# rampasek/GraphGPS

Measured on NVIDIA H100. Metric: graphs/sec GPSLayer fwd+bwd, higher is better.
Workload: dtype f32

## Files before the change

graphgps_b200/csrc/attention.cu:

```cuda
#include "kernels.cuh"

namespace gps {

namespace {

constexpr int kWarpsPerBlock = 4;

__device__ __forceinline__ int find_graph(const int* __restrict__ gptr, int B, int node) {
  int lo = 0, hi = B;
  while (hi - lo > 1) {
    int mid = (lo + hi) >> 1;
    if (gptr[mid] <= node) lo = mid; else hi = mid;
  }
  return lo;
}

template <int LPR>
__device__ __forceinline__ float group_sum(float v) {
#pragma unroll
  for (int o = LPR / 2; o > 0; o >>= 1) v += __shfl_xor_sync(0xffffffffu, v, o);
  return v;
}

__device__ __forceinline__ int warp_max_i(int v) {
#pragma unroll
  for (int o = 16; o > 0; o >>= 1) v = max(v, __shfl_xor_sync(0xffffffffu, v, o));
  return v;
}

struct DropQuad {
  Philox4 r;
  uint32_t thr;
  float keep_scale;
};
__device__ __forceinline__ void drop_quad_refresh(DropQuad& q, float p, uint64_t seed, uint64_t offset, int head, int i, int jl) {
  q.r = philox4x32(seed, offset + (uint64_t)(GPS_SITE_ATTN_P + head), ((uint64_t)i << 20) | (uint64_t)(jl >> 2));
}
__device__ __forceinline__ float drop_quad_scale(const DropQuad& q, int jl) {
  const int k = jl & 3;
  const uint32_t bits = k == 0 ? q.r.v[0] : k == 1 ? q.r.v[1] : k == 2 ? q.r.v[2] : q.r.v[3];
  return bits >= q.thr ? q.keep_scale : 0.f;
}
__device__ __forceinline__ void drop_quad_init(DropQuad& q, float p) {
  q.thr = (uint32_t)fminf(p * 4294967296.f, 4294967295.f);
  q.keep_scale = 1.f / (1.f - p);
}

template <int CH, int LPR>
__device__ __forceinline__ void load_slice(float4* dst, const float* row, int sub, int nch, bool ok) {
#pragma unroll
  for (int c = 0; c < CH; ++c) {
    int ch = sub + c * LPR;
    dst[c] = (ok && ch < nch) ? ld4(row + ch * 4) : f4zero();
  }
}
template <int CH, int LPR>
__device__ __forceinline__ void store_slice(const float4* src, float* row, int sub, int nch) {
#pragma unroll
  for (int c = 0; c < CH; ++c) {
    int ch = sub + c * LPR;
    if (ch < nch) st4(row + ch * 4, src[c]);
  }
}
template <int CH, int LPR>
__device__ __forceinline__ void store_slice_planes(const float4* src, const Planes& p, int64_t r, int64_t col0, int sub, int nch) {
  if (!p.hi) return;
#pragma unroll
  for (int c = 0; c < CH; ++c) {
    int ch = sub + c * LPR;
    if (ch < nch) planes_store4(p, r, col0 + ch * 4, src[c]);
  }
}
template <int CH>
__device__ __forceinline__ float dot_slice(const float4* a, const float4* b) {
  float s = 0.f;
#pragma unroll
  for (int c = 0; c < CH; ++c) s += a[c].x * b[c].x + a[c].y * b[c].y + a[c].z * b[c].z + a[c].w * b[c].w;
  return s;
}

struct AttnArgs {
  const int* gptr; int B; int N; int H; int hd;
  const float* Q; const float* K; const float* V; int64_t ld;
  float* O; const float* Oc; const float* dO; int64_t ldo;
  float* lse; const float* lsec; float* delta; const float* deltac;
  float* dQ; float* dK; float* dV; int64_t ldg;
  float scale; float p_drop; uint64_t seed, offset;
  const unsigned long long* offset_dev;
  Planes Op, dQp, dKp, dVp;
  int smem_rows;
};
__device__ __forceinline__ uint64_t eff_offset(const AttnArgs& a) {
  return a.offset + ((a.p_drop > 0.f && a.offset_dev) ? *a.offset_dev : 0ull);
}

struct StagedRows {
  const float* x; int64_t ldx;
  const float* y; int64_t ldy;
};
template <int RPB>
__device__ __forceinline__ StagedRows stage_rows(const AttnArgs& a, const float* X, int64_t ldX, const float* Y, int64_t ldY,
                                                 int h, float* sm) {
  const int64_t hoff = (int64_t)h * a.hd;
  StagedRows r{X + hoff, ldX, Y + hoff, ldY};
  const int r0 = blockIdx.x * RPB;
  if (a.smem_rows <= 0 || r0 >= a.N) return r;
  const int last = min(r0 + RPB, a.N) - 1;
  const int kmin = a.gptr[find_graph(a.gptr, a.B, r0)];
  const int R = a.gptr[find_graph(a.gptr, a.B, last) + 1] - kmin;
  if (R > a.smem_rows) return r;
  const int pitch = a.hd + 4, nch = a.hd >> 2;
  float* sx = sm;
  float* sy = sm + (int64_t)a.smem_rows * pitch;
  for (int idx = threadIdx.x; idx < R * nch; idx += blockDim.x) {
    const int row = idx / nch, c = idx - row * nch;
    st4(sx + row * pitch + c * 4, ld4(X + (int64_t)(kmin + row) * ldX + hoff + c * 4));
    st4(sy + row * pitch + c * 4, ld4(Y + (int64_t)(kmin + row) * ldY + hoff + c * 4));
  }
  __syncthreads();
  r.x = sx - (int64_t)kmin * pitch; r.ldx = pitch;
  r.y = sy - (int64_t)kmin * pitch; r.ldy = pitch;
  return r;
}

template <int CH, int LPR>
__global__ void __launch_bounds__(kWarpsPerBlock * 32) k_attn_fwd(AttnArgs a) {
  extern __shared__ float attn_sm[];
  constexpr int RPW = 32 / LPR;
  const int warp = threadIdx.x >> 5, lane = threadIdx.x & 31;
  const int sub = lane % LPR, rloc = lane / LPR;
  const int h = blockIdx.y;
  const int i = (blockIdx.x * kWarpsPerBlock + warp) * RPW + rloc;
  const bool row_ok = i < a.N;
  const int nch = a.hd / 4;
  const uint64_t offs = eff_offset(a);
  int gs = 0, n = 0;
  if (row_ok) {
    int g = find_graph(a.gptr, a.B, i);
    gs = a.gptr[g];
    n = a.gptr[g + 1] - gs;
  }
  const int nloop = warp_max_i(n);
  const int64_t hoff = (int64_t)h * a.hd;
  float4 q[CH], o[CH];
  load_slice<CH, LPR>(q, a.Q + (int64_t)(row_ok ? i : 0) * a.ld + hoff, sub, nch, row_ok);
#pragma unroll
  for (int c = 0; c < CH; ++c) {
    q[c] = f4scale(q[c], a.scale);
    o[c] = f4zero();
  }
  float m = -INFINITY, l = 0.f;
  const bool use_drop = a.p_drop > 0.f;
  DropQuad dq;
  drop_quad_init(dq, a.p_drop);
  const StagedRows kv = stage_rows<RPW * kWarpsPerBlock>(a, a.K, a.ld, a.V, a.ld, h, attn_sm);
  float4 kc[CH], vc[CH];
  load_slice<CH, LPR>(kc, kv.x + (int64_t)gs * kv.ldx, sub, nch, n > 0);
  load_slice<CH, LPR>(vc, kv.y + (int64_t)gs * kv.ldy, sub, nch, n > 0);
  for (int jl = 0; jl < nloop; ++jl) {
    if (use_drop && (jl & 3) == 0) drop_quad_refresh(dq, a.p_drop, a.seed, offs, h, i, jl);
    const bool valid = jl < n;
    const bool nvalid = jl + 1 < n;
    const int jn = gs + (nvalid ? jl + 1 : 0);
    float4 kn[CH], vn[CH];
    load_slice<CH, LPR>(kn, kv.x + (int64_t)jn * kv.ldx, sub, nch, nvalid);
    load_slice<CH, LPR>(vn, kv.y + (int64_t)jn * kv.ldy, sub, nch, nvalid);
    float s = group_sum<LPR>(dot_slice<CH>(q, kc));
    s = valid ? s : -INFINITY;
    const float m_new = fmaxf(m, s);
    const float corr = (m_new == -INFINITY) ? 1.f : __expf(m - m_new);
    const float p = valid ? __expf(s - m_new) : 0.f;
    l = l * corr + p;
    const float pd = use_drop ? p * drop_quad_scale(dq, jl) : p;
#pragma unroll
    for (int c = 0; c < CH; ++c) {
      o[c].x = o[c].x * corr + pd * vc[c].x;
      o[c].y = o[c].y * corr + pd * vc[c].y;
      o[c].z = o[c].z * corr + pd * vc[c].z;
      o[c].w = o[c].w * corr + pd * vc[c].w;
      kc[c] = kn[c];
      vc[c] = vn[c];
    }
    m = m_new;
  }
  if (row_ok) {
    const float inv = 1.f / l;
#pragma unroll
    for (int c = 0; c < CH; ++c) o[c] = f4scale(o[c], inv);
    store_slice<CH, LPR>(o, a.O + (int64_t)i * a.ldo + hoff, sub, nch);
    store_slice_planes<CH, LPR>(o, a.Op, i, hoff, sub, nch);
    if (sub == 0) a.lse[(int64_t)i * a.H + h] = m + __logf(l);
  }
}

__global__ void k_attn_delta(AttnArgs a) {
  const int64_t t = ((int64_t)blockIdx.x * blockDim.x + threadIdx.x) >> 3;
  const int sub = threadIdx.x & 7;
  const bool ok = t < (int64_t)a.N * a.H;
  const int64_t i = ok ? t / a.H : 0;
  const int h = ok ? (int)(t - i * a.H) : 0;
  const float4* go = reinterpret_cast<const float4*>(a.dO + i * a.ldo + (int64_t)h * a.hd);
  const float4* oo = reinterpret_cast<const float4*>(a.Oc + i * a.ldo + (int64_t)h * a.hd);
  float acc = 0.f;
  if (ok)
    for (int c = sub; c < a.hd / 4; c += 8) {
      const float4 x = __ldg(go + c), y = __ldg(oo + c);
      acc += x.x * y.x + x.y * y.y + x.z * y.z + x.w * y.w;
    }
  acc += __shfl_xor_sync(0xffffffffu, acc, 4);
  acc += __shfl_xor_sync(0xffffffffu, acc, 2);
  acc += __shfl_xor_sync(0xffffffffu, acc, 1);
  if (ok && sub == 0) a.delta[t] = acc;
}

template <int CH, int LPR>
__device__ __forceinline__ void attn_bwd_q_body(const AttnArgs& a, float* attn_sm) {
  constexpr int RPW = 32 / LPR;
  const int warp = threadIdx.x >> 5, lane = threadIdx.x & 31;
  const int sub = lane % LPR, rloc = lane / LPR;
  const int h = blockIdx.y;
  const int i = (blockIdx.x * kWarpsPerBlock + warp) * RPW + rloc;
  const bool row_ok = i < a.N;
  const int nch = a.hd / 4;
  const uint64_t offs = eff_offset(a);
  int gs = 0, n = 0;
  if (row_ok) {
    int g = find_graph(a.gptr, a.B, i);
    gs = a.gptr[g];
    n = a.gptr[g + 1] - gs;
  }
  const int nloop = warp_max_i(n);
  const int64_t hoff = (int64_t)h * a.hd;
  const int ir = row_ok ? i : 0;
  float4 q[CH], go[CH], gq[CH];
  load_slice<CH, LPR>(q, a.Q + (int64_t)ir * a.ld + hoff, sub, nch, row_ok);
  load_slice<CH, LPR>(go, a.dO + (int64_t)ir * a.ldo + hoff, sub, nch, row_ok);
  {
    const float dl = row_ok ? a.deltac[(int64_t)i * a.H + h] : 0.f;
#pragma unroll
    for (int c = 0; c < CH; ++c) gq[c] = f4zero();
    const float lse = row_ok ? a.lsec[(int64_t)i * a.H + h] : 0.f;
#pragma unroll
    for (int c = 0; c < CH; ++c) q[c] = f4scale(q[c], a.scale);
    const bool use_drop = a.p_drop > 0.f;
    DropQuad dq;
    drop_quad_init(dq, a.p_drop);
    const StagedRows kv = stage_rows<RPW * kWarpsPerBlock>(a, a.K, a.ld, a.V, a.ld, h, attn_sm);
    float4 kk[CH], vv[CH];
    load_slice<CH, LPR>(kk, kv.x + (int64_t)gs * kv.ldx, sub, nch, n > 0);
    load_slice<CH, LPR>(vv, kv.y + (int64_t)gs * kv.ldy, sub, nch, n > 0);
    for (int jl = 0; jl < nloop; ++jl) {
      if (use_drop && (jl & 3) == 0) drop_quad_refresh(dq, a.p_drop, a.seed, offs, h, i, jl);
      const bool valid = jl < n;
      const bool nvalid = jl + 1 < n;
      const int jn = gs + (nvalid ? jl + 1 : 0);
      float4 kn[CH], vn[CH];
      load_slice<CH, LPR>(kn, kv.x + (int64_t)jn * kv.ldx, sub, nch, nvalid);
      load_slice<CH, LPR>(vn, kv.y + (int64_t)jn * kv.ldy, sub, nch, nvalid);
      float s = dot_slice<CH>(q, kk), dp = dot_slice<CH>(go, vv);
#pragma unroll
      for (int ofs = LPR / 2; ofs > 0; ofs >>= 1) {
        s += __shfl_xor_sync(0xffffffffu, s, ofs);
        dp += __shfl_xor_sync(0xffffffffu, dp, ofs);
      }
      const float p = valid ? __expf(s - lse) : 0.f;
      const float ds = p * (dp * (use_drop ? drop_quad_scale(dq, jl) : 1.f) - dl);
#pragma unroll
      for (int c = 0; c < CH; ++c) {
        gq[c].x += ds * kk[c].x;
        gq[c].y += ds * kk[c].y;
        gq[c].z += ds * kk[c].z;
        gq[c].w += ds * kk[c].w;
        kk[c] = kn[c];
        vv[c] = vn[c];
      }
    }
  }
  if (row_ok) {
#pragma unroll
    for (int c = 0; c < CH; ++c) gq[c] = f4scale(gq[c], a.scale);
    store_slice<CH, LPR>(gq, a.dQ + (int64_t)i * a.ldg + hoff, sub, nch);
    store_slice_planes<CH, LPR>(gq, a.dQp, i, hoff, sub, nch);
  }
}

template <int CH, int LPR>
__device__ __forceinline__ void attn_bwd_kv_body(const AttnArgs& a, float* attn_sm) {
  constexpr int RPW = 32 / LPR;
  const int warp = threadIdx.x >> 5, lane = threadIdx.x & 31;
  const int sub = lane % LPR, rloc = lane / LPR;
  const int h = blockIdx.y;
  const int j = (blockIdx.x * kWarpsPerBlock + warp) * RPW + rloc;
  const bool row_ok = j < a.N;
  const int nch = a.hd / 4;
  const uint64_t offs = eff_offset(a);
  int gs = 0, n = 0;
  if (row_ok) {
    int g = find_graph(a.gptr, a.B, j);
    gs = a.gptr[g];
    n = a.gptr[g + 1] - gs;
  }
  const int nloop = warp_max_i(n);
  const int jl = j - gs;
  const int64_t hoff = (int64_t)h * a.hd;
  const int jr = row_ok ? j : 0;
  float4 kk[CH], vv[CH], gk[CH], gv[CH];
  load_slice<CH, LPR>(kk, a.K + (int64_t)jr * a.ld + hoff, sub, nch, row_ok);
  load_slice<CH, LPR>(vv, a.V + (int64_t)jr * a.ld + hoff, sub, nch, row_ok);
#pragma unroll
  for (int c = 0; c < CH; ++c) {
    gk[c] = f4zero();
    gv[c] = f4zero();
  }
  const StagedRows qd = stage_rows<RPW * kWarpsPerBlock>(a, a.Q, a.ld, a.dO, a.ldo, h, attn_sm);
  float4 q[CH], go[CH];
  load_slice<CH, LPR>(q, qd.x + (int64_t)gs * qd.ldx, sub, nch, n > 0);
  load_slice<CH, LPR>(go, qd.y + (int64_t)gs * qd.ldy, sub, nch, n > 0);
  for (int il = 0; il < nloop; ++il) {
    const bool valid = il < n;
    const int i = gs + (valid ? il : 0);
    const bool nvalid = il + 1 < n;
    const int in_ = gs + (nvalid ? il + 1 : 0);
    float4 qn[CH], gon[CH];
    load_slice<CH, LPR>(qn, qd.x + (int64_t)in_ * qd.ldx, sub, nch, nvalid);
    load_slice<CH, LPR>(gon, qd.y + (int64_t)in_ * qd.ldy, sub, nch, nvalid);
    float s = dot_slice<CH>(q, kk), dp = dot_slice<CH>(go, vv);
#pragma unroll
    for (int ofs = LPR / 2; ofs > 0; ofs >>= 1) {
      s += __shfl_xor_sync(0xffffffffu, s, ofs);
      dp += __shfl_xor_sync(0xffffffffu, dp, ofs);
    }
    const float lse = valid ? a.lsec[(int64_t)i * a.H + h] : 0.f;
    const float dl = valid ? a.deltac[(int64_t)i * a.H + h] : 0.f;
    const float p = valid ? __expf(s * a.scale - lse) : 0.f;
    float dsc = 1.f;
    if (a.p_drop > 0.f) {
      DropQuad dq;
      drop_quad_init(dq, a.p_drop);
      drop_quad_refresh(dq, a.p_drop, a.seed, offs, h, i, jl);
      dsc = drop_quad_scale(dq, jl);
    }
    const float pd = p * dsc;
    const float ds = p * (dp * dsc - dl) * a.scale;
#pragma unroll
    for (int c = 0; c < CH; ++c) {
      gk[c].x += ds * q[c].x; gk[c].y += ds * q[c].y; gk[c].z += ds * q[c].z; gk[c].w += ds * q[c].w;
      gv[c].x += pd * go[c].x; gv[c].y += pd * go[c].y; gv[c].z += pd * go[c].z; gv[c].w += pd * go[c].w;
      q[c] = qn[c];
      go[c] = gon[c];
    }
  }
  if (row_ok) {
    store_slice<CH, LPR>(gk, a.dK + (int64_t)j * a.ldg + hoff, sub, nch);
    store_slice<CH, LPR>(gv, a.dV + (int64_t)j * a.ldg + hoff, sub, nch);
    store_slice_planes<CH, LPR>(gk, a.dKp, j, hoff, sub, nch);
    store_slice_planes<CH, LPR>(gv, a.dVp, j, hoff, sub, nch);
  }
}

template <int CH, int LPR>
__global__ void __launch_bounds__(kWarpsPerBlock * 32) k_attn_bwd(AttnArgs a) {
  extern __shared__ float attn_sm[];
  if (blockIdx.z == 0) attn_bwd_kv_body<CH, LPR>(a, attn_sm);
  else attn_bwd_q_body<CH, LPR>(a, attn_sm);
}

enum { KFWD = 0, KBWD = 1 };

constexpr int kStageBytes = 72 * 1024;

template <int CH, int LPR>
static void launch_one(int which, const AttnArgs& a0, cudaStream_t stream) {
  constexpr int RPW = 32 / LPR;
  AttnArgs a = a0;
  static const bool stage_on = [] {
    const char* e = getenv("GPS_B200_ATTN_STAGE");
    return e && e[0] == '1';
  }();
  const int pitch = a.hd + 4;
  a.smem_rows = (stage_on && a.B > 0 && a.N < 64LL * a.B) ? kStageBytes / (2 * pitch * 4) : 0;
  const size_t smem = a.smem_rows > 0 ? (size_t)2 * a.smem_rows * pitch * 4 : 0;
  static bool attr_done[2] = {false, false};
  if (smem > 0 && !attr_done[which]) {
    if (which == KFWD) cudaFuncSetAttribute(k_attn_fwd<CH, LPR>, cudaFuncAttributeMaxDynamicSharedMemorySize, kStageBytes);
    else cudaFuncSetAttribute(k_attn_bwd<CH, LPR>, cudaFuncAttributeMaxDynamicSharedMemorySize, kStageBytes);
    attr_done[which] = true;
  }
  dim3 grid((unsigned)ceil_div(a.N, (int64_t)RPW * kWarpsPerBlock), (unsigned)a.H, which == KFWD ? 1 : 2);
  dim3 block(kWarpsPerBlock * 32);
  if (which == KFWD) k_attn_fwd<CH, LPR><<<grid, block, smem, stream>>>(a);
  else k_attn_bwd<CH, LPR><<<grid, block, smem, stream>>>(a);
}

static int dispatch(int which, const AttnArgs& a, cudaStream_t stream) {
  GPS_REQUIRE(a.hd > 0 && a.hd % 4 == 0, GPS_ERR_UNSUPPORTED, "attention: head dim %d must be a multiple of 4", a.hd);
  GPS_REQUIRE(a.ld % 4 == 0 && a.ldo % 4 == 0 && (which == KFWD || a.ldg % 4 == 0), GPS_ERR_UNSUPPORTED,
              "attention: leading dimensions must be multiples of 4");
  const int nch = a.hd / 4;
  GPS_REQUIRE(nch <= 48, GPS_ERR_UNSUPPORTED, "attention: head dim %d > 192 not supported", a.hd);
  if (a.N == 0) return GPS_OK;
  int lpr = 1;
  while ((nch + lpr - 1) / lpr > 6) lpr *= 2;
  const int ch = (nch + lpr - 1) / lpr;
#define GPS_ATTN_CASE(CHV, LPRV)                                  \
  if (ch == CHV && lpr == LPRV) {                                 \
    launch_one<CHV, LPRV>(which, a, stream);                      \
    GPS_LAUNCH_CHECK();                                           \
    return GPS_OK;                                                \
  }
  GPS_ATTN_CASE(1, 1) GPS_ATTN_CASE(2, 1) GPS_ATTN_CASE(3, 1) GPS_ATTN_CASE(4, 1) GPS_ATTN_CASE(5, 1)
  GPS_ATTN_CASE(6, 1) GPS_ATTN_CASE(4, 2) GPS_ATTN_CASE(5, 2) GPS_ATTN_CASE(6, 2) GPS_ATTN_CASE(4, 4)
  GPS_ATTN_CASE(5, 4) GPS_ATTN_CASE(6, 4) GPS_ATTN_CASE(4, 8) GPS_ATTN_CASE(5, 8) GPS_ATTN_CASE(6, 8)
#undef GPS_ATTN_CASE
  set_error("attention: no kernel for head dim %d", a.hd);
  return GPS_ERR_UNSUPPORTED;
}

}

int attention_fwd(const GpsGraph& g, int64_t heads, int64_t hd, const float* Q, const float* K, const float* V,
                  int64_t ld, float* O, int64_t ldo, float* lse, float p_drop, uint64_t seed, uint64_t offset,
                  cudaStream_t stream, const unsigned long long* offset_dev, Planes Op) {
  AttnArgs a{};
  a.offset_dev = offset_dev;
  a.Op = Op;
  a.gptr = g.graph_ptr; a.B = (int)g.B; a.N = (int)g.N; a.H = (int)heads; a.hd = (int)hd;
  a.Q = Q; a.K = K; a.V = V; a.ld = ld; a.O = O; a.ldo = ldo; a.lse = lse;
  a.scale = 1.f / sqrtf((float)hd); a.p_drop = p_drop; a.seed = seed; a.offset = offset;
  return dispatch(KFWD, a, stream);
}

int attention_bwd(const GpsGraph& g, int64_t heads, int64_t hd, const float* Q, const float* K, const float* V,
                  int64_t ld, const float* O, const float* dO, int64_t ldo, const float* lse, float* delta,
                  float* dQ, float* dK, float* dV, int64_t ldg, float p_drop, uint64_t seed, uint64_t offset,
                  cudaStream_t stream, const unsigned long long* offset_dev, Planes dQp, Planes dKp, Planes dVp) {
  AttnArgs a{};
  a.offset_dev = offset_dev;
  a.dQp = dQp; a.dKp = dKp; a.dVp = dVp;
  a.gptr = g.graph_ptr; a.B = (int)g.B; a.N = (int)g.N; a.H = (int)heads; a.hd = (int)hd;
  a.Q = Q; a.K = K; a.V = V; a.ld = ld; a.Oc = O; a.dO = dO; a.ldo = ldo; a.lsec = lse;
  a.delta = delta; a.deltac = delta; a.dQ = dQ; a.dK = dK; a.dV = dV; a.ldg = ldg;
  a.scale = 1.f / sqrtf((float)hd); a.p_drop = p_drop; a.seed = seed; a.offset = offset;
  if (a.N == 0) return GPS_OK;
  const int64_t nt = (int64_t)a.N * a.H * 8;
  k_attn_delta<<<(unsigned)ceil_div(nt, (int64_t)256), 256, 0, stream>>>(a);
  GPS_LAUNCH_CHECK();
  return dispatch(KBWD, a, stream);
}

}
```

graphgps_b200/csrc/layer.cu:

```cuda
#include <stdarg.h>
#include <string.h>

#include <algorithm>
#include <atomic>

#include "gemm.cuh"
#include "kernels.cuh"

namespace gps {

int perf_supported(int64_t dim_head, int64_t features);
int64_t perf_mp();
int perf_prep(const float* P, int64_t m, float* Pn, const GpsGraph& g, int64_t H, int* nmax, float* gmax, int* argk,
              cudaStream_t st);
int perf_features_fwd(float* fq, float* fk, const float* Q, const float* K, const GpsGraph& g, int64_t H, int64_t m,
                      float* gmax, int* argq, int* argk, cudaStream_t st);
int perf_linattn_fwd(const GpsGraph& g, int64_t H, int64_t m, const int* nmax, const float* qf, const float* kf,
                     const float* V, const float* gmax, float* O, cudaStream_t st);
int perf_linattn_bwd(const GpsGraph& g, int64_t H, int64_t m, const int* nmax, const float* qf, const float* kf,
                     const float* V, const float* gmax, const float* gO, float* g_qf, float* g_kf, float* gV,
                     float* ggmax, cudaStream_t st);
int perf_features_bwd(float* g_fq, float* g_fk, const float* fq, const float* fk, const float* Q, const float* K,
                      float* gQ, float* gK, const GpsGraph& g, int64_t H, int64_t m, const int* argq, const int* argk,
                      float* ggmax, cudaStream_t st);
// ... 778 lines not shown
    const Planes wp[3] = {P.pq_p, P.pk_p, P.pv_p};
    float* dst[3] = {P.pQ, P.pK, P.pV};
    for (int i = 0; i < 3; ++i)
      GPS_TRY(gemm(linear_fwd(P, N, inner, d, {a->x, d, P.x_p}, {lin[i]->weight, d, wp[i]}, dst[i], inner), sg));
    GPS_TRY(perf_prep(a->perf_proj, P.m, P.pPn, a->graph, P.H, P.pnmax, P.pgmax, P.pargk, sg));
    float* ddst[2] = {P.pfq, P.pfk};
    for (int i = 0; i < 2; ++i)
      GPS_TRY(gemm(linear_fwd(P, NH, P.mp, dh, {dst[i], dh}, {P.pPn, dh}, ddst[i], P.mp), sg));
    GPS_TRY(perf_features_fwd(P.pfq, P.pfk, P.pQ, P.pK, a->graph, P.H, P.m, P.pgmax, P.pargq, P.pargk, sg));
    if (P.perf_pairwise)
      GPS_TRY(perf_quad_fwd(a->graph, P.H, P.m, P.pnmax, P.pfq, P.pfk, P.pV, P.pgmax, P.O, P.pden, sg));
    else
      GPS_TRY(perf_linattn_fwd(a->graph, P.H, P.m, P.pnmax, P.pfq, P.pfk, P.pV, P.pgmax, P.O, sg));
    GemmParams g = linear_fwd(P, N, d, inner, {P.O, inner}, {a->attn_out.weight, inner}, P.hA, d, a->attn_out.bias);
    g.R1 = a->x; g.ldr1 = (int)d; g.stats = stats(BN_A);
    set_dropout(g, P.drop(GPS_SITE_ATTN_OUT));
    g.p_drop2 = P.pa; g.site2 = GPS_SITE_PERF_OUT;
    if (P.nonorm) GPS_TRY(close_with_s(g, sg));
    GPS_TRY(gemm(g, sg));
  }

  if (two_branches) GPS_TRY(sd->order(sd->s3, st));

  if (!P.nonorm) {
    const bool loc = P.gated || P.gine || P.gcn;
    const float* first = loc ? P.xloc : P.hA;
    BnView bf = loc ? bn_view(P, BN_L, a->norm1_local, N) : bn_view(P, BN_A, a->norm1_attn, N);
    const float* second = (loc && (P.attn || P.perf)) ? P.hA : nullptr;
    BnView bs = bn_view(P, BN_A, a->norm1_attn, N);
    GPS_TRY(bn_combine(first, bf, second, bs, P.s, N, d, st, P.s_p));
  }

  {
    GemmParams g = linear_fwd(P, N, 2 * d, d, {P.s, d, P.s_p}, {a->ff1.weight, d, P.ff1_p}, P.hid, 2 * d, a->ff1.bias);
    g.act = act; g.C_pre = P.hid_pre; g.ldpre = (int)(2 * d); g.Cp = P.hid_p;
    set_dropout(g, P.drop(GPS_SITE_FF1));
    GPS_TRY(gemm(g, st));
    GemmParams g2 = linear_fwd(P, N, d, 2 * d, {P.hid, 2 * d, P.hid_p}, {a->ff2.weight, 2 * d, P.ff2_p}, P.t, d,
                               a->ff2.bias);
    g2.R1 = P.s; g2.ldr1 = (int)d; g2.stats = stats(BN_2);
    set_dropout(g2, P.drop(GPS_SITE_FF2));
    if (P.nonorm) {
      g2.C = a->x_out;
      g2.Cp = out_planes(a->x_planes_out);
    }
    GPS_TRY(gemm(g2, st));
    if (!P.nonorm)
      GPS_TRY(bn_combine(P.t, bn_view(P, BN_2, a->norm2, N), nullptr, BnView(), a->x_out, N, d, st,
                         out_planes(a->x_planes_out)));
  }
  return GPS_OK;
}

static int layer_backward(const GpsLayerArgs* a, cudaStream_t st) {
  Plan P;
  GPS_TRY(make_plan(a, &P, true));
  GPS_REQUIRE(a->saved && a->workspace, GPS_ERR_ARG, "saved/workspace buffers are required");
  GPS_REQUIRE(a->workspace_bytes >= P.bwd_bytes, GPS_ERR_ARG, "workspace too small (%lld < %lld)",
              (long long)a->workspace_bytes, (long long)P.bwd_bytes);
  GPS_TRY(check_params(a, P));
  GPS_REQUIRE(a->grad_x_out && a->grad_x, GPS_ERR_ARG, "grad_x_out / grad_x are required");
  const int64_t N = P.N, E = P.E, d = P.d;
  const int act = a->act;
  DropCfg nodrop;
  auto sums = [&](int which) { return P.bsums + (int64_t)which * 2 * d; };
  GPS_CUDA(cudaMemsetAsync(P.bsums, 0, (size_t)P.nbn * 2 * d * sizeof(double), st));
  Side* sd;
  GPS_TRY(side_stream(&sd));
  cudaStream_t s2 = sd->s;
  auto wfork = [&](cudaStream_t from) -> int { return sd->order(from, s2); };
  const bool two_branches = (P.gated || P.gine || P.gcn) && (P.attn || P.perf);
  cudaStream_t sa = two_branches ? sd->s3 : st;
  cudaStream_t se = sd->s4;
  const int opt = opt_flags();
  auto record_ev = [&](void* ev, cudaStream_t s) -> int {
    if (!ev) return GPS_OK;
    cudaStreamCaptureStatus cs = cudaStreamCaptureStatusNone;
    GPS_CUDA(cudaStreamIsCapturing(s, &cs));
    GPS_CUDA(cudaEventRecordWithFlags((cudaEvent_t)ev, s, cs == cudaStreamCaptureStatusActive ? cudaEventRecordExternal
                                                                                               : cudaEventRecordDefault));
    return GPS_OK;
  };
  auto early_done = [&]() -> int { return record_ev(a->ev_grads_early, s2); };
  auto mid_done = [&]() -> int { return record_ev(a->ev_grads_mid, s2); };
  const bool gx_splitk = P.Wy >= 1024 && N > 0;
  if (P.Wy) {
    GPS_TRY(wfork(st));
    GPS_CUDA(cudaMemsetAsync(P.gWcat, 0, (size_t)(P.Wy * d + P.Wy) * sizeof(float), s2));
  }
  if (gx_splitk) GPS_CUDA(cudaMemsetAsync(a->grad_x, 0, (size_t)(N * d) * sizeof(float), st));

  if (P.gated) {
    GPS_TRY(sd->order(st, se));
    BnView ve = bn_view(P, BN_E, a->bn_edge_e);
    if (a->grad_edge_out && E > 0) {
      GPS_TRY(bn_bwd_reduce(a->grad_edge_out, d, P.ehat, d, E, d, ve, act, P.drop(GPS_SITE_GCN_E), sums(BN_E), se));
      GPS_TRY(bn_bwd_apply(a->grad_edge_out, d, P.ehat, d, E, d, ve, act, P.drop(GPS_SITE_GCN_E), sums(BN_E), P.g_e, d,
                           a->bn_edge_e.grad_weight, a->bn_edge_e.grad_bias, se, P.grads_accumulate));
    } else {
      if (E > 0) GPS_CUDA(cudaMemsetAsync(P.g_e, 0, (size_t)(E * d) * sizeof(float), se));
      if (a->bn_edge_e.grad_weight && !P.grads_prezeroed)
        GPS_CUDA(cudaMemsetAsync(a->bn_edge_e.grad_weight, 0, d * sizeof(float), se));
      if (a->bn_edge_e.grad_bias && !P.grads_prezeroed)
        GPS_CUDA(cudaMemsetAsync(a->bn_edge_e.grad_bias, 0, d * sizeof(float), se));
    }
  }

  const float* g_t = P.nonorm ? a->grad_x_out : P.g_t;
  if (!P.nonorm) {
    BnView v2 = bn_view(P, BN_2, a->norm2);
    GPS_TRY(bn_bwd_reduce(a->grad_x_out, d, P.t, d, N, d, v2, -1, nodrop, sums(BN_2), st));
    GPS_TRY(bn_bwd_apply(a->grad_x_out, d, P.t, d, N, d, v2, -1, nodrop, sums(BN_2), P.g_t, d, a->norm2.grad_weight,
                         a->norm2.grad_bias, st, P.grads_accumulate, P.gt_p));
  } else if (!(P.dropout.p > 0.f) && P.gt_p.hi && N > 0) {
    ToPlanesItem it{g_t, d, (int)N, (int)d, P.gt_p};
    GPS_TRY(to_planes(&it, 1, st));
  }
  const float* g_xloc = P.nonorm ? P.g_s : P.g_xloc;
  const Planes g_xloc_p = P.nonorm ? P.gs_p : P.gl1_p;
  const float* g_hA = P.nonorm ? P.g_s : P.g_hA;
  const Planes g_hA_p = P.nonorm ? P.gs_p : P.ghA_p;

  bool fused_la = false;
  {
    Operand g_ff2;
    GPS_TRY(dropmul(P, {g_t, d, P.gt_p}, P.g_tmp, P.gtmp_p, GPS_SITE_FF2, st, &g_ff2));
    GemmParams g = linear_dgrad(P, N, 2 * d, d, g_ff2, {a->ff2.weight, 2 * d, P.ff2_p}, P.g_hid, 2 * d);
    set_act_mask(g, act, P.hid, P.hid_pre, 2 * d);
    set_dropout(g, P.drop(GPS_SITE_FF1));
    g.Cp = P.ghid_p;
    GPS_TRY(gemm(g, st));
    const Operand g_hid{P.g_hid, 2 * d, P.ghid_p};
    GPS_TRY(wfork(st));
    GPS_TRY(linear_wgrad(P, g_ff2, {P.hid, 2 * d, P.hid_p}, N, d, 2 * d, a->ff2.grad_weight, a->ff2.grad_bias, s2));
    GPS_TRY(linear_wgrad(P, g_hid, {P.s, d, P.s_p}, N, 2 * d, d, a->ff1.grad_weight, a->ff1.grad_bias, s2));
    GemmParams g2 = linear_dgrad(P, N, d, 2 * d, g_hid, {a->ff1.weight, d, P.ff1_p}, P.g_s, d);
    g2.R1 = g_t; g2.ldr1 = (int)d;
    g2.Cp = P.gs_p;
    fused_la = (opt & 64) && !P.nonorm && P.use_planes && g2.Ap.hi && g2.Bp.hi && N > 0 && P.train;
    if (fused_la) {
      if (P.gated || P.gine || P.gcn) {
        BnView v = bn_view(P, BN_L, a->norm1_local);
        g2.bnred[0].z = P.xloc; g2.bnred[0].ldz = (int)d; g2.bnred[0].mean = v.mean; g2.bnred[0].invstd = v.invstd;
        g2.bnred[0].sums = sums(BN_L);
      }
      if (P.attn || P.perf) {
        BnView v = bn_view(P, BN_A, a->norm1_attn);
        g2.bnred[1].z = P.hA; g2.bnred[1].ldz = (int)d; g2.bnred[1].mean = v.mean; g2.bnred[1].invstd = v.invstd;
        g2.bnred[1].sums = sums(BN_A);
      }
    }
    GPS_TRY(gemm(g2, st));
  }

  const bool loc = P.gated || P.gine || P.gcn;
  bool chain_x = false;
  if (loc && !P.nonorm) {
    BnView v = bn_view(P, BN_L, a->norm1_local);
    if (!fused_la) GPS_TRY(bn_bwd_reduce(P.g_s, d, P.xloc, d, N, d, v, -1, nodrop, sums(BN_L), st));
    chain_x = P.gated && N > 0 && (opt & 32) && P.train;
    if (chain_x)
      GPS_TRY(bn_bwd_apply_chain(P.g_s, d, P.xloc, d, N, d, v, sums(BN_L), P.g_xloc, d, a->norm1_local.grad_weight,
                                 a->norm1_local.grad_bias, P.grads_accumulate, P.gl1_p, P.xt, d,
                                 bn_view(P, BN_X, a->bn_node_x), act, P.drop(GPS_SITE_GCN_X), sums(BN_X), st));
    else
      GPS_TRY(bn_bwd_apply(P.g_s, d, P.xloc, d, N, d, v, -1, nodrop, sums(BN_L), P.g_xloc, d,
                           a->norm1_local.grad_weight, a->norm1_local.grad_bias, st, P.grads_accumulate, P.gl1_p));
  }
  if (!P.attn && !P.perf) {
    GPS_TRY(wfork(st));
    GPS_TRY(early_done());
  }
  if (two_branches) GPS_TRY(sd->order(st, sa));
  if (P.attn) {
    if (!P.nonorm) {
      BnView v = bn_view(P, BN_A, a->norm1_attn);
      if (!fused_la) GPS_TRY(bn_bwd_reduce(P.g_s, d, P.hA, d, N, d, v, -1, nodrop, sums(BN_A), sa));
      GPS_TRY(bn_bwd_apply(P.g_s, d, P.hA, d, N, d, v, -1, nodrop, sums(BN_A), P.g_hA, d, a->norm1_attn.grad_weight,
                           a->norm1_attn.grad_bias, sa, P.grads_accumulate, P.ghA_p));
    }
    Operand g_ao;
    GPS_TRY(dropmul(P, {g_hA, d, g_hA_p}, P.g_tmp2, P.gtmp2_p, GPS_SITE_ATTN_OUT, sa, &g_ao));
    GPS_TRY(gemm(linear_dgrad(P, N, d, d, g_ao, {a->attn_out.weight, d, P.out_p}, P.g_O, d), sa));
    GPS_TRY(wfork(sa));
    GPS_TRY(linear_wgrad(P, g_ao, {P.O, d, P.O_p}, N, d, d, a->attn_out.grad_weight, a->attn_out.grad_bias, s2));
    GPS_TRY(early_done());
    const float* Q = P.Y1 + P.qkv_off;
    float* gQ = P.gY1 + P.qkv_off;
    GPS_TRY(attention_bwd(a->graph, P.H, P.hd, Q, Q + d, Q + 2 * d, P.Wy, P.O, P.g_O, d, P.lse, P.delta, gQ, gQ + d,
                          gQ + 2 * d, P.Wy, P.pa, a->seed, a->offset, sa, (const unsigned long long*)a->offset_dev,
                          P.gY1_p.cols(P.qkv_off), P.gY1_p.cols(P.qkv_off + d), P.gY1_p.cols(P.qkv_off + 2 * d)));
  }

  if (P.perf) {
    const int64_t inner = P.inner, NH = N * P.H, dh = a->perf_dim_head;
    if (!P.nonorm) {
      BnView v = bn_view(P, BN_A, a->norm1_attn);
      if (!fused_la) GPS_TRY(bn_bwd_reduce(P.g_s, d, P.hA, d, N, d, v, -1, nodrop, sums(BN_A), sa));
      GPS_TRY(bn_bwd_apply(P.g_s, d, P.hA, d, N, d, v, -1, nodrop, sums(BN_A), P.g_hA, d, a->norm1_attn.grad_weight,
                           a->norm1_attn.grad_bias, sa, P.grads_accumulate));
    }
    Operand g_ao;
    GPS_TRY(dropmul(P, {g_hA, d}, P.g_tmp2, Planes(), GPS_SITE_ATTN_OUT, sa, &g_ao, P.pa, GPS_SITE_PERF_OUT));
    GPS_TRY(gemm(linear_dgrad(P, N, inner, d, g_ao, {a->attn_out.weight, inner}, P.g_O, inner), sa));
    GPS_TRY(wfork(sa));
    GPS_TRY(linear_wgrad(P, g_ao, {P.O, inner}, N, d, inner, a->attn_out.grad_weight, a->attn_out.grad_bias, s2));
    GPS_TRY(early_done());
    if (P.perf_pairwise)
      GPS_TRY(perf_quad_bwd(a->graph, P.H, P.m, P.pnmax, P.pfq, P.pfk, P.pV, P.pgmax, P.O, P.pden, P.g_O, P.g_pden,
                            P.g_pfq, P.g_pfk, P.g_pV, P.g_pgmax, sa));
    else
      GPS_TRY(perf_linattn_bwd(a->graph, P.H, P.m, P.pnmax, P.pfq, P.pfk, P.pV, P.pgmax, P.g_O, P.g_pfq, P.g_pfk, P.g_pV,
                               P.g_pgmax, sa));
    GPS_TRY(perf_features_bwd(P.g_pfq, P.g_pfk, P.pfq, P.pfk, P.pQ, P.pK, P.g_pQ, P.g_pK, a->graph, P.H, P.m, P.pargq,
                              P.pargk, P.g_pgmax, sa));
    float* gdd[2] = {P.g_pfq, P.g_pfk};
    float* gqk[2] = {P.g_pQ, P.g_pK};
    for (int i = 0; i < 2; ++i) {
      GemmParams h = linear_dgrad(P, NH, dh, P.mp, {gdd[i], P.mp}, {P.pPn, dh}, gqk[i], dh);
      h.R1 = gqk[i]; h.ldr1 = (int)dh;
      GPS_TRY(gemm(h, sa));
    }
    const GpsLinear* lin[3] = {&a->perf_q, &a->perf_k, &a->perf_v};
    const float* gsrc[3] = {P.g_pQ, P.g_pK, P.g_pV};
    GPS_TRY(wfork(sa));
    for (int i = 0; i < 3; ++i) {
      GPS_TRY(linear_wgrad(P, {gsrc[i], inner}, {a->x, d}, N, inner, d, lin[i]->grad_weight, nullptr, s2));
      GemmParams h = linear_dgrad(P, N, d, inner, {gsrc[i], inner}, {lin[i]->weight, d}, P.g_xp, d);
      h.R1 = i == 0 ? g_hA : P.g_xp; h.ldr1 = (int)d;
      GPS_TRY(gemm(h, sa));
    }
  }

  const float* g_x_local = nullptr;
  if (P.gated) {
    BnView vx = bn_view(P, BN_X, a->bn_node_x);
    if (!chain_x)
      GPS_TRY(bn_bwd_reduce(g_xloc, d, P.xt, d, N, d, vx, act, P.drop(GPS_SITE_GCN_X), sums(BN_X), st));
    GPS_TRY(bn_bwd_apply(g_xloc, d, P.xt, d, N, d, vx, act, P.drop(GPS_SITE_GCN_X), sums(BN_X), P.gY1, P.Wy,
                         a->bn_node_x.grad_weight, a->bn_node_x.grad_bias, st, P.grads_accumulate, P.gY1_p));
    GPS_TRY(sd->order(se, st));
    GPS_TRY(gatedgcn_bwd_dst(a->graph, d, P.gY1, P.Wy, P.ehat, P.Y1 + d, P.Wy, P.g_e, P.g_num, P.gY1 + 2 * d, st, P.ge_p,
                             P.gY1_p.cols(2 * d), P.pe_rho, P.g_den));
    if (P.eslap) {
      GPS_TRY(sd->order(st, se));
      GPS_TRY(eslap_bwd(a->graph, a->pe, a->pe_dim, d, act, P.g_num, P.g_den, P.Y1 + d, P.Wy, P.ehat, P.pe_r, P.pe_rho,
                        a->pe_mlp0.weight, a->pe_mlp0.bias, a->pe_mlp1.weight, P.pe_gz, P.pe_gr, P.pe_part, a->grad_pe,
                        a->pe_mlp0.grad_weight, a->pe_mlp0.grad_bias, a->pe_mlp1.grad_weight, a->pe_mlp1.grad_bias,
                        P.grads_accumulate, se));
    }
    GPS_TRY(gatedgcn_bwd_src(a->graph, d, P.g_e, P.ehat, P.g_num, P.gY1 + 3 * d, P.gY1 + d, P.Wy, st, P.gY1_p.cols(3 * d),
                             P.gY1_p.cols(d), P.pe_rho));
    const Operand g_e{P.g_e, d, P.ge_p};
    GPS_TRY(wfork(st));
    GPS_TRY(linear_wgrad(P, g_e, {a->edge_attr, d, P.e_p}, E, d, d, a->gcn_C.grad_weight, a->gcn_C.grad_bias, s2));
    if (P.eslap) GPS_TRY(sd->order(se, s2));
    GPS_TRY(mid_done());
    if (a->grad_edge_attr && E > 0) {
      GemmParams g = linear_dgrad(P, E, d, d, g_e, {a->gcn_C.weight, d, P.C_p}, a->grad_edge_attr, d);
      g.R1 = a->grad_edge_out; g.ldr1 = (int)d;
      GPS_TRY(gemm(g, st));
    }
    g_x_local = g_xloc;
  } else if (P.gine) {
    Operand g_l1;
    GPS_TRY(dropmul(P, {g_xloc, d, g_xloc_p}, P.g_tmp3, P.gtmp3_p, GPS_SITE_LOCAL, st, &g_l1));
    GemmParams g = linear_dgrad(P, N, d, d, g_l1, {a->gine_lin1.weight, d, P.g1_p}, P.g_h1, d);
    set_act_mask(g, act, P.h1, P.h1_pre, d);
    g.Cp = P.gh1_p;
    GPS_TRY(gemm(g, st));
    const Operand g_h1{P.g_h1, d, P.gh1_p};
    GPS_TRY(wfork(st));
    GPS_TRY(linear_wgrad(P, g_l1, {P.h1, d, P.h1_p}, N, d, d, a->gine_lin1.grad_weight, a->gine_lin1.grad_bias, s2));
    GPS_TRY(linear_wgrad(P, g_h1, {P.agg, d, P.agg_p}, N, d, d, a->gine_lin0.grad_weight, a->gine_lin0.grad_bias, s2));
    GPS_TRY(mid_done());
    GPS_TRY(gemm(linear_dgrad(P, N, d, d, g_h1, {a->gine_lin0.weight, d, P.g0_p}, P.g_agg, d), st));
    GPS_REQUIRE(a->grad_edge_attr || E == 0, GPS_ERR_ARG, "grad_edge_attr is required for GINE");
    GPS_TRY(gine_bwd_dst(a->graph, d, a->x, a->edge_attr, P.g_agg, a->grad_edge_attr, st));
    GPS_TRY(gine_bwd_src(a->graph, d, a->grad_edge_attr, P.g_agg, a->gine_eps, g_xloc, P.g_xl, st));
    g_x_local = P.g_xl;
  } else if (P.gcn) {
    Operand g_h;
    GPS_TRY(dropmul(P, {g_xloc, d}, P.g_tmp3, Planes(), GPS_SITE_LOCAL, st, &g_h));
    if (a->gcn_conv.grad_bias) {
      if (!P.grads_prezeroed) GPS_CUDA(cudaMemsetAsync(a->gcn_conv.grad_bias, 0, (size_t)d * sizeof(float), st));
      GPS_TRY(colsum(g_h.f, d, N, d, a->gcn_conv.grad_bias, st));
    }
    GPS_TRY(gcn_bwd(a->graph, d, g_h.f, P.dinv, P.gY1, P.Wy, st, P.gY1_p));
    GPS_TRY(wfork(st));
    GPS_TRY(mid_done());
    g_x_local = g_xloc;
  }

  if (two_branches) GPS_TRY(sd->order(sa, st));

  if (P.Wy) {
    const Operand gY1{P.gY1, P.Wy, P.gY1_p};
    GPS_TRY(wfork(st));
    GPS_TRY(wgrad_add(P, gY1, {a->x, d, P.x_p}, N, P.Wy, d, P.gWcat, P.gbcat, s2));
    PackDesc pdsc = pack_desc(P);
    k_unpack<<<(unsigned)P.Wy, 128, 0, s2>>>(pdsc, P.gWcat, P.gbcat, P.grads_accumulate ? 1 : 0);
    GPS_LAUNCH_CHECK();
    GemmParams g = linear_dgrad(P, N, d, P.Wy, gY1, {P.Wcat, d, P.Wcat_p}, a->grad_x, d);
    g.R1 = g_x_local; g.ldr1 = (int)d;
    g.R2 = P.attn ? g_hA : (P.perf ? P.g_xp : nullptr); g.ldr2 = (int)d;
    if (gx_splitk) g.splitk = 4;
    GPS_TRY(gemm(g, st));
  } else if (g_x_local) {
    GPS_TRY(add3(g_x_local, d, P.perf ? P.g_xp : nullptr, d, nullptr, 0, a->grad_x, d, N, d, st));
  } else {
    GPS_TRY(add3(P.g_xp, d, nullptr, 0, nullptr, 0, a->grad_x, d, N, d, st));
  }
  GPS_TRY(sd->join(st));
  GPS_TRY(record_ev(a->ev_grads_done, st));
  return GPS_OK;
}

}

using namespace gps;

extern "C" const char* gps_last_error(void) { return g_err; }
extern "C" int gps_abi_version(void) { return GPS_ABI_VERSION; }
extern "C" const char* gps_build_arch(void) { return "sm_90a"; }
extern "C" unsigned long long gps_launch_count(void) { return g_launches.load(); }
extern "C" unsigned long long gps_fallback_count(void) { return g_fallbacks.load(); }
// ... 233 lines not shown
```

Measured before the change: 338,900.

## Add fused shared-memory attention backward kernel for small graphs

```diff
diff --git a/graphgps_b200/csrc/attention.cu b/graphgps_b200/csrc/attention.cu
--- a/graphgps_b200/csrc/attention.cu
+++ b/graphgps_b200/csrc/attention.cu
@@ -6,13 +6,15 @@
 
 constexpr int kWarpsPerBlock = 4;
 
-__device__ __forceinline__ int find_graph(const int* __restrict__ gptr, int B, int node) {
-  int lo = 0, hi = B;
+__device__ __forceinline__ int find_graph_in(const int* __restrict__ gptr, int lo, int hi, int node) {
   while (hi - lo > 1) {
     int mid = (lo + hi) >> 1;
     if (gptr[mid] <= node) lo = mid; else hi = mid;
   }
   return lo;
+}
+__device__ __forceinline__ int find_graph(const int* __restrict__ gptr, int B, int node) {
+  return find_graph_in(gptr, 0, B, node);
 }
 
 template <int LPR>
@@ -214,13 +216,8 @@
 }
 
 template <int CH, int LPR>
-__device__ __forceinline__ void attn_bwd_q_body(const AttnArgs& a, float* attn_sm) {
-  constexpr int RPW = 32 / LPR;
-  const int warp = threadIdx.x >> 5, lane = threadIdx.x & 31;
-  const int sub = lane % LPR, rloc = lane / LPR;
-  const int h = blockIdx.y;
-  const int i = (blockIdx.x * kWarpsPerBlock + warp) * RPW + rloc;
-  const bool row_ok = i < a.N;
+__device__ __forceinline__ void attn_bwd_q_body(const AttnArgs& a, int h, int i, bool row_ok) {
+  const int sub = (threadIdx.x & 31) % LPR;
   const int nch = a.hd / 4;
   const uint64_t offs = eff_offset(a);
   int gs = 0, n = 0;
@@ -245,18 +242,19 @@
     const bool use_drop = a.p_drop > 0.f;
     DropQuad dq;
     drop_quad_init(dq, a.p_drop);
-    const StagedRows kv = stage_rows<RPW * kWarpsPerBlock>(a, a.K, a.ld, a.V, a.ld, h, attn_sm);
+    const float* Kh = a.K + hoff;
+    const float* Vh = a.V + hoff;
     float4 kk[CH], vv[CH];
-    load_slice<CH, LPR>(kk, kv.x + (int64_t)gs * kv.ldx, sub, nch, n > 0);
-    load_slice<CH, LPR>(vv, kv.y + (int64_t)gs * kv.ldy, sub, nch, n > 0);
+    load_slice<CH, LPR>(kk, Kh + (int64_t)gs * a.ld, sub, nch, n > 0);
+    load_slice<CH, LPR>(vv, Vh + (int64_t)gs * a.ld, sub, nch, n > 0);
     for (int jl = 0; jl < nloop; ++jl) {
       if (use_drop && (jl & 3) == 0) drop_quad_refresh(dq, a.p_drop, a.seed, offs, h, i, jl);
       const bool valid = jl < n;
       const bool nvalid = jl + 1 < n;
       const int jn = gs + (nvalid ? jl + 1 : 0);
       float4 kn[CH], vn[CH];
-      load_slice<CH, LPR>(kn, kv.x + (int64_t)jn * kv.ldx, sub, nch, nvalid);
-      load_slice<CH, LPR>(vn, kv.y + (int64_t)jn * kv.ldy, sub, nch, nvalid);
+      load_slice<CH, LPR>(kn, Kh + (int64_t)jn * a.ld, sub, nch, nvalid);
+      load_slice<CH, LPR>(vn, Vh + (int64_t)jn * a.ld, sub, nch, nvalid);
       float s = dot_slice<CH>(q, kk), dp = dot_slice<CH>(go, vv);
 #pragma unroll
       for (int ofs = LPR / 2; ofs > 0; ofs >>= 1) {
@@ -285,13 +283,8 @@
 }
 
 template <int CH, int LPR>
-__device__ __forceinline__ void attn_bwd_kv_body(const AttnArgs& a, float* attn_sm) {
-  constexpr int RPW = 32 / LPR;
-  const int warp = threadIdx.x >> 5, lane = threadIdx.x & 31;
-  const int sub = lane % LPR, rloc = lane / LPR;
-  const int h = blockIdx.y;
-  const int j = (blockIdx.x * kWarpsPerBlock + warp) * RPW + rloc;
-  const bool row_ok = j < a.N;
+__device__ __forceinline__ void attn_bwd_kv_body(const AttnArgs& a, int h, int j, bool row_ok) {
+  const int sub = (threadIdx.x & 31) % LPR;
   const int nch = a.hd / 4;
   const uint64_t offs = eff_offset(a);
   int gs = 0, n = 0;
@@ -312,18 +305,19 @@
     gk[c] = f4zero();
     gv[c] = f4zero();
   }
-  const StagedRows qd = stage_rows<RPW * kWarpsPerBlock>(a, a.Q, a.ld, a.dO, a.ldo, h, attn_sm);
+  const float* Qh = a.Q + hoff;
+  const float* dOh = a.dO + hoff;
   float4 q[CH], go[CH];
-  load_slice<CH, LPR>(q, qd.x + (int64_t)gs * qd.ldx, sub, nch, n > 0);
-  load_slice<CH, LPR>(go, qd.y + (int64_t)gs * qd.ldy, sub, nch, n > 0);
+  load_slice<CH, LPR>(q, Qh + (int64_t)gs * a.ld, sub, nch, n > 0);
+  load_slice<CH, LPR>(go, dOh + (int64_t)gs * a.ldo, sub, nch, n > 0);
   for (int il = 0; il < nloop; ++il) {
     const bool valid = il < n;
     const int i = gs + (valid ? il : 0);
     const bool nvalid = il + 1 < n;
     const int in_ = gs + (nvalid ? il + 1 : 0);
     float4 qn[CH], gon[CH];
-    load_slice<CH, LPR>(qn, qd.x + (int64_t)in_ * qd.ldx, sub, nch, nvalid);
-    load_slice<CH, LPR>(gon, qd.y + (int64_t)in_ * qd.ldy, sub, nch, nvalid);
+    load_slice<CH, LPR>(qn, Qh + (int64_t)in_ * a.ld, sub, nch, nvalid);
+    load_slice<CH, LPR>(gon, dOh + (int64_t)in_ * a.ldo, sub, nch, nvalid);
     float s = dot_slice<CH>(q, kk), dp = dot_slice<CH>(go, vv);
 #pragma unroll
     for (int ofs = LPR / 2; ofs > 0; ofs >>= 1) {
@@ -360,12 +354,176 @@
 
 template <int CH, int LPR>
 __global__ void __launch_bounds__(kWarpsPerBlock * 32) k_attn_bwd(AttnArgs a) {
+  constexpr int RPW = 32 / LPR;
+  const int i = (blockIdx.x * kWarpsPerBlock + (threadIdx.x >> 5)) * RPW + (threadIdx.x & 31) / LPR;
+  if (blockIdx.z == 0) attn_bwd_kv_body<CH, LPR>(a, blockIdx.y, i, i < a.N);
+  else attn_bwd_q_body<CH, LPR>(a, blockIdx.y, i, i < a.N);
+}
+
+__host__ __device__ constexpr int bwd_small_pitch(int hd) { return ((hd >> 2) & 1) ? hd : hd + 4; }
+__host__ __device__ constexpr int64_t bwd_small_smem_bytes(int hd, int rows) {
+  return 4 * ((int64_t)rows * (4 * bwd_small_pitch(hd) + hd / 4 + 2) + 2LL * rows * (rows + 1));
+}
+constexpr int kBwdSmallSmemBytes = 44 * 1024;
+
+__device__ __forceinline__ int warp_first_above(const int* __restrict__ gptr, int lo, int hi, int x) {
+  const int lane = threadIdx.x & 31;
+  while (hi > lo) {
+    const int step = (hi - lo + 30) / 31;
+    const unsigned above = __ballot_sync(0xffffffffu, gptr[min(lo + lane * step, hi)] > x);
+    const int f = __ffs(above) - 1;
+    if (f == 0) return lo;
+    hi = min(lo + f * step, hi);
+    lo += (f - 1) * step + 1;
+  }
+  return lo;
+}
+
+__device__ __forceinline__ float dot4(float4 a, float4 b) { return a.x * b.x + a.y * b.y + a.z * b.z + a.w * b.w; }
+__device__ __forceinline__ float4 f4axpy(float w, float4 x, float4 y) {
+  return make_float4(fmaf(w, x.x, y.x), fmaf(w, x.y, y.y), fmaf(w, x.z, y.z), fmaf(w, x.w, y.w));
+}
+
+template <int LPR>
+__global__ void __launch_bounds__(kWarpsPerBlock * 32) k_attn_bwd_small(AttnArgs a) {
   extern __shared__ float attn_sm[];
-  if (blockIdx.z == 0) attn_bwd_kv_body<CH, LPR>(a, attn_sm);
-  else attn_bwd_q_body<CH, LPR>(a, attn_sm);
-}
-
-enum { KFWD = 0, KBWD = 1 };
+  __shared__ int s_nmax;
+  constexpr int NT = kWarpsPerBlock * 32;
+  const int rows = a.smem_rows, hd = a.hd, nch = hd >> 2, pitch = bwd_small_pitch(hd);
+  const int h = blockIdx.y;
+  const int64_t hoff = (int64_t)h * hd;
+  float* sQ = attn_sm;
+  float* sK = sQ + rows * pitch;
+  float* sV = sK + rows * pitch;
+  float* sdO = sV + rows * pitch;
+  float* sPart = sdO + rows * pitch;
+  int* sG0 = reinterpret_cast<int*>(sPart + rows * nch);
+  int* sN = sG0 + rows;
+  float* sPd = reinterpret_cast<float*>(sN + rows);
+  float* sDs = sPd + rows * (rows + 1);
+
+  const int win = (rows + 1) / 2;
+  const int r0 = blockIdx.x * win, r1 = min(r0 + win, a.N);
+  const int gb = warp_first_above(a.gptr, 0, a.B, r0 - 1), ge = warp_first_above(a.gptr, 0, a.B, r1 - 1);
+  const float scale = a.scale;
+  const bool use_drop = a.p_drop > 0.f;
+  DropQuad dq;
+  drop_quad_init(dq, a.p_drop);
+  const uint64_t offs = eff_offset(a);
+  if (threadIdx.x == 0) s_nmax = 0;
+  __syncthreads();
+
+  for (int g = gb; g < ge;) {
+    const int a0 = a.gptr[g];
+    const int k = a.gptr[ge] <= a0 + rows ? ge : warp_first_above(a.gptr, g, ge, a0 + rows) - 1;
+    if (k == g) {
+      constexpr int RPW = 32 / LPR;
+      const int e0 = a.gptr[g + 1];
+      const int warp = threadIdx.x >> 5, lane = threadIdx.x & 31;
+      for (int i = a0 + warp; i < e0; i += kWarpsPerBlock) {
+        float acc = 0.f;
+        for (int c = lane; c < nch; c += 32)
+          acc += dot4(ld4(a.dO + (int64_t)i * a.ldo + hoff + 4 * c), ld4(a.Oc + (int64_t)i * a.ldo + hoff + 4 * c));
+#pragma unroll
+        for (int o = 16; o > 0; o >>= 1) acc += __shfl_xor_sync(0xffffffffu, acc, o);
+        if (lane == 0) a.delta[(int64_t)i * a.H + h] = acc;
+      }
+      __syncthreads();
+      for (int base = a0; base < e0; base += RPW * kWarpsPerBlock) {
+        const int i = base + warp * RPW + lane / LPR;
+        attn_bwd_q_body<2, LPR>(a, h, i, i < e0);
+        attn_bwd_kv_body<2, LPR>(a, h, i, i < e0);
+      }
+      ++g;
+      continue;
+    }
+    const int gfirst = g;
+    const int R = a.gptr[k] - a0;
+    g = k;
+    if (R == 0) continue;
+
+    for (int r = threadIdx.x; r < R; r += NT) {
+      const int gg = find_graph_in(a.gptr, gfirst, k, a0 + r);
+      const int s0 = a.gptr[gg], n = a.gptr[gg + 1] - s0;
+      sG0[r] = s0 - a0;
+      sN[r] = n;
+      atomicMax(&s_nmax, n);
+    }
+#pragma unroll 2
+    for (int idx = threadIdx.x; idx < R * nch; idx += NT) {
+      const int r = idx / nch, c = idx - r * nch;
+      const int64_t i = a0 + r;
+      const int64_t qo = i * a.ld + hoff + 4 * c, oo = i * a.ldo + hoff + 4 * c;
+      const float4 go = ld4(a.dO + oo);
+      st4(sQ + r * pitch + 4 * c, ld4(a.Q + qo));
+      st4(sK + r * pitch + 4 * c, ld4(a.K + qo));
+      st4(sV + r * pitch + 4 * c, ld4(a.V + qo));
+      st4(sdO + r * pitch + 4 * c, go);
+      sPart[idx] = dot4(go, ld4(a.Oc + oo));
+    }
+    __syncthreads();
+
+    const int nmax = s_nmax | 1, nq = (s_nmax + 3) >> 2;
+    for (int idx = threadIdx.x; idx < R * nq; idx += NT) {
+      const int qd = idx / R, r = idx - qd * R;
+      const int n = sN[r], j0 = 4 * qd;
+      if (j0 >= n) continue;
+      const int i = a0 + r;
+      const float lse = a.lsec[(int64_t)i * a.H + h];
+      const float* kb = sK + sG0[r] * pitch;
+      const float* vb = sV + sG0[r] * pitch;
+      int jo[4];
+#pragma unroll
+      for (int t = 0; t < 4; ++t) jo[t] = min(j0 + t, n - 1) * pitch;
+      float s[4] = {0.f, 0.f, 0.f, 0.f}, dp[4] = {0.f, 0.f, 0.f, 0.f};
+      for (int c = 0; c < nch; ++c) {
+        const float4 q = ld4(sQ + r * pitch + 4 * c), go = ld4(sdO + r * pitch + 4 * c);
+#pragma unroll
+        for (int t = 0; t < 4; ++t) {
+          s[t] += dot4(q, ld4(kb + jo[t] + 4 * c));
+          dp[t] += dot4(go, ld4(vb + jo[t] + 4 * c));
+        }
+      }
+      float dl = 0.f;
+      for (int c = 0; c < nch; ++c) dl += sPart[r * nch + c];
+      if (use_drop) drop_quad_refresh(dq, a.p_drop, a.seed, offs, h, i, j0);
+#pragma unroll
+      for (int t = 0; t < 4; ++t) {
+        const int jl = j0 + t;
+        if (jl < n) {
+          const float p = __expf(s[t] * scale - lse);
+          const float m = use_drop ? drop_quad_scale(dq, jl) : 1.f;
+          sPd[r * nmax + jl] = p * m;
+          sDs[r * nmax + jl] = p * (dp[t] * m - dl) * scale;
+        }
+      }
+    }
+    __syncthreads();
+
+    for (int idx = threadIdx.x; idx < R * nch; idx += NT) {
+      const int r = idx / nch, c = idx - r * nch;
+      const int g0 = sG0[r], n = sN[r], jr = r - g0;
+      float4 gq = f4zero(), gk = f4zero(), gv = f4zero();
+      for (int t = 0; t < n; ++t) {
+        const int row = g0 + t;
+        gq = f4axpy(sDs[r * nmax + t], ld4(sK + row * pitch + 4 * c), gq);
+        gk = f4axpy(sDs[row * nmax + jr], ld4(sQ + row * pitch + 4 * c), gk);
+        gv = f4axpy(sPd[row * nmax + jr], ld4(sdO + row * pitch + 4 * c), gv);
+      }
+      const int64_t i = a0 + r, col = hoff + 4 * c;
+      st4(a.dQ + i * a.ldg + col, gq);
+      st4(a.dK + i * a.ldg + col, gk);
+      st4(a.dV + i * a.ldg + col, gv);
+      if (a.dQp.hi) planes_store4(a.dQp, i, col, gq);
+      if (a.dKp.hi) planes_store4(a.dKp, i, col, gk);
+      if (a.dVp.hi) planes_store4(a.dVp, i, col, gv);
+    }
+    if (threadIdx.x == 0) s_nmax = 0;
+    __syncthreads();
+  }
+}
+
+enum { KFWD = 0, KBWD = 1, KBWD_SMALL = 2 };
 
 constexpr int kStageBytes = 72 * 1024;
 
@@ -373,21 +531,20 @@
 static void launch_one(int which, const AttnArgs& a0, cudaStream_t stream) {
   constexpr int RPW = 32 / LPR;
   AttnArgs a = a0;
+  dim3 block(kWarpsPerBlock * 32);
   static const bool stage_on = [] {
     const char* e = getenv("GPS_B200_ATTN_STAGE");
     return e && e[0] == '1';
   }();
   const int pitch = a.hd + 4;
-  a.smem_rows = (stage_on && a.B > 0 && a.N < 64LL * a.B) ? kStageBytes / (2 * pitch * 4) : 0;
+  a.smem_rows = (which == KFWD && stage_on && a.B > 0 && a.N < 64LL * a.B) ? kStageBytes / (2 * pitch * 4) : 0;
   const size_t smem = a.smem_rows > 0 ? (size_t)2 * a.smem_rows * pitch * 4 : 0;
-  static bool attr_done[2] = {false, false};
-  if (smem > 0 && !attr_done[which]) {
-    if (which == KFWD) cudaFuncSetAttribute(k_attn_fwd<CH, LPR>, cudaFuncAttributeMaxDynamicSharedMemorySize, kStageBytes);
-    else cudaFuncSetAttribute(k_attn_bwd<CH, LPR>, cudaFuncAttributeMaxDynamicSharedMemorySize, kStageBytes);
-    attr_done[which] = true;
+  static bool attr_done = false;
+  if (smem > 0 && !attr_done) {
+    cudaFuncSetAttribute(k_attn_fwd<CH, LPR>, cudaFuncAttributeMaxDynamicSharedMemorySize, kStageBytes);
+    attr_done = true;
   }
   dim3 grid((unsigned)ceil_div(a.N, (int64_t)RPW * kWarpsPerBlock), (unsigned)a.H, which == KFWD ? 1 : 2);
-  dim3 block(kWarpsPerBlock * 32);
   if (which == KFWD) k_attn_fwd<CH, LPR><<<grid, block, smem, stream>>>(a);
   else k_attn_bwd<CH, LPR><<<grid, block, smem, stream>>>(a);
 }
@@ -399,6 +556,25 @@
   const int nch = a.hd / 4;
   GPS_REQUIRE(nch <= 48, GPS_ERR_UNSUPPORTED, "attention: head dim %d > 192 not supported", a.hd);
   if (a.N == 0) return GPS_OK;
+  if (which == KBWD_SMALL) {
+    AttnArgs b = a;
+    b.smem_rows = 1;
+    while (bwd_small_smem_bytes(a.hd, b.smem_rows + 1) <= kBwdSmallSmemBytes) ++b.smem_rows;
+    const dim3 grid((unsigned)ceil_div(a.N, (int64_t)(b.smem_rows + 1) / 2), (unsigned)a.H), block(kWarpsPerBlock * 32);
+    const size_t smem = (size_t)bwd_small_smem_bytes(a.hd, b.smem_rows);
+    int lpr = 1;
+    while ((nch + lpr - 1) / lpr > 2) lpr *= 2;
+    switch (lpr) {
+      case 1: k_attn_bwd_small<1><<<grid, block, smem, stream>>>(b); break;
+      case 2: k_attn_bwd_small<2><<<grid, block, smem, stream>>>(b); break;
+      case 4: k_attn_bwd_small<4><<<grid, block, smem, stream>>>(b); break;
+      case 8: k_attn_bwd_small<8><<<grid, block, smem, stream>>>(b); break;
+      case 16: k_attn_bwd_small<16><<<grid, block, smem, stream>>>(b); break;
+      default: k_attn_bwd_small<32><<<grid, block, smem, stream>>>(b); break;
+    }
+    GPS_LAUNCH_CHECK();
+    return GPS_OK;
+  }
   int lpr = 1;
   while ((nch + lpr - 1) / lpr > 6) lpr *= 2;
   const int ch = (nch + lpr - 1) / lpr;
@@ -442,6 +618,7 @@
   a.delta = delta; a.deltac = delta; a.dQ = dQ; a.dK = dK; a.dV = dV; a.ldg = ldg;
   a.scale = 1.f / sqrtf((float)hd); a.p_drop = p_drop; a.seed = seed; a.offset = offset;
   if (a.N == 0) return GPS_OK;
+  if (a.B > 0 && a.N < 64LL * a.B) return dispatch(KBWD_SMALL, a, stream);
   const int64_t nt = (int64_t)a.N * a.H * 8;
   k_attn_delta<<<(unsigned)ceil_div(nt, (int64_t)256), 256, 0, stream>>>(a);
   GPS_LAUNCH_CHECK();
diff --git a/graphgps_b200/csrc/layer.cu b/graphgps_b200/csrc/layer.cu
--- a/graphgps_b200/csrc/layer.cu
+++ b/graphgps_b200/csrc/layer.cu
@@ -954,6 +954,7 @@
     }
     GPS_TRY(gemm(g2, st));
   }
+  if (two_branches) GPS_TRY(sd->order(st, sa));
 
   const bool loc = P.gated || P.gine || P.gcn;
   bool chain_x = false;
@@ -969,11 +970,11 @@
       GPS_TRY(bn_bwd_apply(P.g_s, d, P.xloc, d, N, d, v, -1, nodrop, sums(BN_L), P.g_xloc, d,
                            a->norm1_local.grad_weight, a->norm1_local.grad_bias, st, P.grads_accumulate, P.gl1_p));
   }
+  if (two_branches && !P.nonorm) GPS_TRY(wfork(st));
   if (!P.attn && !P.perf) {
     GPS_TRY(wfork(st));
     GPS_TRY(early_done());
   }
-  if (two_branches) GPS_TRY(sd->order(st, sa));
   if (P.attn) {
     if (!P.nonorm) {
       BnView v = bn_view(P, BN_A, a->norm1_attn);
```

New measurement: 348,900 (median of 6 runs). +3.0%, better.
